# XinShuo-ph/gaussian_splatting_with_eye_tracking

Hardware: AMD Instinct MI355X
Metric: rendered views/sec (fwd+bwd) at 1080p, 1M Gaussians; achieved HBM GB/s % (higher is better)
Workload: dtype fp32; 1 GPU

## Files before the change

### gaussian_splatting_with_eye_tracking_amd/csrc/backward.hip

```cpp
#include <algorithm>

#include <hip/hip_ext.h>

#include "gs_blend.cuh"
#include "gs_blend_bwd.cuh"
#include "gs_bwd_math.cuh"
#include "gs_device.cuh"
#include "gs_kernels.h"

namespace gsamd {

constexpr int kDefaultBwdVariant = 2;
int g_bwd_variant = kDefaultBwdVariant;
void set_backward_variant(int v) { g_bwd_variant = v == 0 ? 0 : kDefaultBwdVariant; }

static BlendBwdParams blend_bwd_params(int W, int H, const ImageView& img, const BinningView& b, const GeomView& g,
                                       const float* colors, const float* bg, const float* dL_dpix) {
    return BlendBwdParams{W, H, img.ranges, img.max_contrib, b.point_list, reinterpret_cast<const float2*>(g.means2D),
                          reinterpret_cast<const float4*>(g.conic_opacity), colors, img.accum_alpha, img.n_contrib,
                          dL_dpix, bg, g.grad_accum, g_cull, (W + 15) / 16, img.bucket_count, img.bucket_list, g.hdr};
}

void launch_render_backward(int W, int H, const ImageView& img, const BinningView& b, const GeomView& g,
                            const float* colors, const float* bg, const float* dL_dpix, hipStream_t s) {
    const int gx = (W + 15) / 16, gy = (H + 15) / 16;
    if (gx == 0 || gy == 0) return;
    const BlendBwdParams p = blend_bwd_params(W, H, img, b, g, colors, bg, dL_dpix);
    const DispatchEvents ev = take_dispatch_events();
    if (g_bwd_variant == 0)
        hipExtLaunchKernelGGL(render_bwd_rows_kernel<BwdRows::kBase>, dim3(gx * gy), dim3(64), 0, s, ev.start, ev.stop,
                              0, p);
    else
        hipExtLaunchKernelGGL(render_bwd_kernel, dim3(gx * gy), dim3(64), 0, s, ev.start, ev.stop, 0, p);
}

constexpr uint32_t kDetNone = 0xffffffffu;
__global__ void __launch_bounds__(256) reduce_partials_kernel(
    int P, uint32_t R, uint32_t gx, uint32_t gy, const int* __restrict__ radii, const float2* __restrict__ means2D,
    const float* __restrict__ depths, const uint32_t* __restrict__ tiles_touched, const uint32_t* __restrict__ ranges,
    const uint32_t* __restrict__ max_contrib, const uint32_t* __restrict__ point_list,
    const float* __restrict__ partials, float* __restrict__ grad_accum, uint32_t* __restrict__ hdr,
    uint32_t err_token) {
    const int p = (int)((blockIdx.x * 256u + threadIdx.x) >> 4);
    const int sub = threadIdx.x & 15;
    if (p >= P) return;
    const int rad = radii[p];
    if (rad <= 0) return;
    const float2 xy = means2D[p];
    const Rect r = get_rect(xy.x, xy.y, rad, 16, 16, gx, gy);
    const uint32_t w = r.x1 - r.x0;
    const uint32_t area = w * (r.y1 - r.y0);
    const uint64_t key = ((uint64_t)float_bits(depths[p]) << 32) | (uint32_t)p;
    bool bad = area != tiles_touched[p];
    double acc = 0.0;
    if (!bad) {
        for (uint32_t i0 = 0; i0 < area; i0 += 16) {
            uint32_t pos = kDetNone;
            const uint32_t i = i0 + (uint32_t)sub;
            if (i < area) {
                const uint32_t tile = (r.y0 + i / w) * gx + r.x0 + i % w;
// ... 69 lines not shown
    const int idx = (int)(blockIdx.x * 256u + threadIdx.x);
    if (idx >= P || radii[idx] <= 0) return;
    float dz = grad_accum[(size_t)idx * kGradRow + kAuxDz];
    if (inv_depths) {
        const float f = inv_depth(inv_depths[idx]);
        dz = -(f * f) * dz;
    }
    dL_dmean3D[3 * idx + 0] += dz * viewmatrix[2];
    dL_dmean3D[3 * idx + 1] += dz * viewmatrix[6];
    dL_dmean3D[3 * idx + 2] += dz * viewmatrix[10];
}

void launch_aux_depth_to_means(int P, const GeomView& g, const int* radii, const float* viewmatrix,
                               float* dL_dmean3D, hipStream_t s, bool inverse) {
    if (P <= 0) return;
    hipLaunchKernelGGL(aux_depth_to_means_kernel, dim3(((unsigned)P + 255u) / 256u), dim3(256), 0, s, P, radii,
                       g.grad_accum, viewmatrix, dL_dmean3D, inverse ? g.depths : nullptr);
}

void launch_amr_render_backward(int W, int H, int mode, const ImageView& img, const BinningView& b,
                                const GeomView& g, const float* colors, const float* bg, const float* dL_dpix,
                                hipStream_t s) {
    const int tgx = (W + 31) / 32, tgy = (H + 31) / 32;
    if (tgx == 0 || tgy == 0 || mode == 0) return;
    BlendBwdParams p = blend_bwd_params(W, H, img, b, g, colors, bg, dL_dpix);
    p.amr_mode = mode;
    p.levels = img.levels;
    p.gx = tgx;
    hipLaunchKernelGGL(render_bwd_rows_kernel<BwdRows::kAmr>, dim3(4 * tgx * tgy), dim3(64), 0, s, p);
}


template <bool kHasSH, bool kHasScales, bool kSH16, bool kDrgb = false, bool kAA = false>
__device__ __forceinline__ void backward_gaussian_body(const BackwardGaussArgs& a,
                                                       const float* __restrict__ grad_accum,
                                                       const uint8_t* __restrict__ clamped_bits, int idx,
                                                       float* lrow, float (*small)[12] = nullptr,
                                                       float (*sh19)[19] = nullptr) {
    if (idx >= a.P) return;
    const bool vis = a.radii[idx] > 0;
    float acc[kNG];
    if (vis) {
        const float4* row = reinterpret_cast<const float4*>(grad_accum + (size_t)idx * kGradRow);
        const float4 r0 = row[0], r1 = row[1];
        const float r2 = grad_accum[(size_t)idx * kGradRow + 8];
        acc[0] = r0.x; acc[1] = r0.y; acc[2] = r0.z; acc[3] = r0.w;
        acc[4] = r1.x; acc[5] = r1.y; acc[6] = r1.z; acc[7] = r1.w; acc[8] = r2;
    } else {
#pragma unroll
        for (int q = 0; q < kNG; q++) acc[q] = 0.f;
    }
    if (a.err_word && (a.hdr[kHdrAntialias] != 0u) != kAA) {
        if (idx == 0) *a.err_word = a.err_token;
        if (vis) {
#pragma unroll
            for (int q = 0; q < kNG; q++) acc[q] = __uint_as_float(0x7fc00000u);
        }
    }
    if (small) {
        (*small)[9] = acc[0];
        (*small)[10] = acc[1];
        (*small)[11] = acc[2];
        (*small)[0] = acc[3];
        (*small)[1] = acc[4];
        (*small)[2] = 0.f;
    } else {
        if (a.dL_dcolor) {
            a.dL_dcolor[3 * idx + 0] = acc[0];
            a.dL_dcolor[3 * idx + 1] = acc[1];
            a.dL_dcolor[3 * idx + 2] = acc[2];
        }
        a.dL_dmean2D[3 * idx + 0] = acc[3];
        a.dL_dmean2D[3 * idx + 1] = acc[4];
        a.dL_dmean2D[3 * idx + 2] = 0.f;
    }
    if (a.dL_dconic) reinterpret_cast<float4*>(a.dL_dconic)[idx] = make_float4(acc[5], acc[6], 0.f, acc[7]);
    if constexpr (!kAA) store_out1(&a.dL_dopacity[idx], acc[8], a.nt_out != 0);

    const int ncoef_out = a.M;
    if (!vis) {
        if constexpr (kAA) store_out1(&a.dL_dopacity[idx], 0.f, a.nt_out != 0);
        if (small) {
#pragma unroll
            for (int i = 3; i < 9; i++) (*small)[i] = 0.f;
        } else {
#pragma unroll
            for (int i = 0; i < 3; i++) a.dL_dmean3D[3 * idx + i] = 0.f;
        }
        if (a.dL_dcov3D) {
#pragma unroll
            for (int i = 0; i < 6; i++) a.dL_dcov3D[6 * idx + i] = 0.f;
        }
        if (kDrgb) {
#pragma unroll
            for (int i = 0; i < 19; i++) (*sh19)[i] = 0.f;
        } else if (kHasSH && kSH16) {
#pragma unroll
            for (int i = 0; i < 48; i++) lrow[i] = 0.f;
        } else if (kHasSH) {
            for (int i = 0; i < ncoef_out * 3; i++) a.dL_dsh[(size_t)idx * ncoef_out * 3 + i] = 0.f;
        }
        if (!small)
            for (int i = 0; i < 3; i++) a.dL_dscale[3 * idx + i] = 0.f;
        for (int i = 0; i < 4; i++) a.dL_drot[4 * idx + i] = 0.f;
        return;
    }

    const float mx = a.means3D[3 * idx], my = a.means3D[3 * idx + 1], mz = a.means3D[3 * idx + 2];
    float cov3D[6];
    float4 qrot = make_float4(0.f, 0.f, 0.f, 0.f);
    float scl[3] = {0.f, 0.f, 0.f};
    if (kHasScales) {
        qrot = reinterpret_cast<const float4*>(a.rotations)[idx];
        scl[0] = a.scales[3 * idx + 0];
        scl[1] = a.scales[3 * idx + 1];
        scl[2] = a.scales[3 * idx + 2];
    }
    if (kHasScales && !a.has_cov_precomp) {
        compute_cov3d(scl, qrot, a.scale_modifier, cov3D);
    } else {
#pragma unroll
        for (int i = 0; i < 6; i++) cov3D[i] = a.cov3D[6 * idx + i];
    }
    float opac = 0.f;
    if constexpr (kAA) opac = a.opacities[idx];
    float s[16][3];
    uint8_t cb = 0;
    const bool use_drgb = kHasSH && a.drgb && a.hdr[kHdrDrgb] == 1u;
    float d9[9];
    if (kHasSH) {
        if (use_drgb) {
            const float4* row = reinterpret_cast<const float4*>(a.drgb) + 3 * (size_t)idx;
            const float4 r0 = row[0], r1 = row[1], r2 = row[2];
            d9[0] = r0.x; d9[1] = r0.y; d9[2] = r0.z; d9[3] = r0.w;
            d9[4] = r1.x; d9[5] = r1.y; d9[6] = r1.z; d9[7] = r1.w; d9[8] = r2.x;
        } else if constexpr (!kDrgb) {
            load_sh_rows<kSH16>(a, idx, s, lrow);
        } else {
// ... 42 lines not shown
        for (int c = 0; c < 3; c++) (*sh19)[16 + c] = dRGB[c];
    } else if (kHasSH) {
        if (use_drgb) sh_backward<kSH16>(a, idx, mx, my, mz, s, cb, acc, dmean, kSH16 ? lrow : nullptr, d9);
        else sh_backward<kSH16>(a, idx, mx, my, mz, s, cb, acc, dmean, kSH16 ? lrow : nullptr, nullptr);
    }
#pragma unroll
    for (int i = 0; i < 3; i++) {
        if (small) (*small)[3 + i] = dmean[i];
        else a.dL_dmean3D[3 * idx + i] = dmean[i];
    }

    if (kHasScales) {
        float dscale[3];
        float4 dq;
        cov3d_backward(qrot, scl, a.scale_modifier, dcov, dscale, dq);
        store_out4(reinterpret_cast<float4*>(a.dL_drot) + idx, dq, a.nt_out != 0);
        if (small) {
            (*small)[6] = dscale[0];
            (*small)[7] = dscale[1];
            (*small)[8] = dscale[2];
        } else {
            a.dL_dscale[3 * idx + 0] = dscale[0];
            a.dL_dscale[3 * idx + 1] = dscale[1];
            a.dL_dscale[3 * idx + 2] = dscale[2];
        }
    } else {
        if (small) {
            (*small)[6] = (*small)[7] = (*small)[8] = 0.f;
        } else {
            for (int i = 0; i < 3; i++) a.dL_dscale[3 * idx + i] = 0.f;
        }
        for (int i = 0; i < 4; i++) a.dL_drot[4 * idx + i] = 0.f;
    }
}

constexpr int kBgStageNt = 16;


template <bool kHasSH, bool kHasScales, bool kSH16, bool kSmall = false, bool kAA = false>
__global__ void __launch_bounds__(256) backward_gaussians_kernel(BackwardGaussArgs a, const float* __restrict__ grad_accum,
                                                                 const uint8_t* __restrict__ clamped_bits, int stage) {
    constexpr bool kStage = kHasSH && kSH16;
    static_assert(!kSmall || kStage, "the small outputs are staged in the SH rows' LDS");
    __shared__ float s_dsh[kStage ? 256 * kShRow : 1];
    const int idx = blockIdx.x * blockDim.x + threadIdx.x;
    if (kStage && !(a.drgb && a.hdr[kHdrDrgb] == 1u)) {
        const int g0 = blockIdx.x * blockDim.x;
        const int n = min(256, a.P - g0);
        const float4* in = reinterpret_cast<const float4*>(a.shs) + (size_t)g0 * 12;
        if (n == 256) {
            float4 v[12];
#pragma unroll
            for (int k = 0; k < 12; k++) v[k] = in[threadIdx.x + 256 * k];
#pragma unroll
            for (int k = 0; k < 12; k++) {
                const int f = threadIdx.x + 256 * k;
                float* r = s_dsh + (f / 12) * kShRow + 4 * (f % 12);
                r[0] = v[k].x; r[1] = v[k].y; r[2] = v[k].z; r[3] = v[k].w;
            }
        } else {
            for (int f = threadIdx.x; f < n * 12; f += 256) {
                const float4 v = in[f];
                float* r = s_dsh + (f / 12) * kShRow + 4 * (f % 12);
                r[0] = v.x; r[1] = v.y; r[2] = v.z; r[3] = v.w;
            }
        }
        __syncthreads();
    }
    float small[12];
    backward_gaussian_body<kHasSH, kHasScales, kSH16, false, kAA>(a, grad_accum, clamped_bits, idx,
                                                                  kStage ? s_dsh + threadIdx.x * kShRow : nullptr,
                                                                  kSmall ? &small : nullptr);
    if constexpr (kStage) {
        __syncthreads();
        const int g0 = blockIdx.x * blockDim.x;
        const int n = min(256, a.P - g0);
        float4* out = reinterpret_cast<float4*>(a.dL_dsh) + (size_t)g0 * 12;
        const bool nt = (stage & kBgStageNt) != 0;
        for (int f = threadIdx.x; f < n * 12; f += 256) {
            const float* r = s_dsh + (f / 12) * kShRow + 4 * (f % 12);
            store_out4(&out[f], make_float4(r[0], r[1], r[2], r[3]), nt);
        }
        if constexpr (kSmall) {
            __syncthreads();
            if (idx < a.P) {
#pragma unroll
                for (int i = 0; i < 12; i++) s_dsh[(i / 3) * 768 + 3 * threadIdx.x + i % 3] = small[i];
            }
            __syncthreads();
            const int nf = 3 * n;
            for (int f = threadIdx.x; f < 4 * 192; f += 256) {
                const int q = f / 192, i = f - 192 * q;
                float* d = q == 0 ? a.dL_dmean2D : q == 1 ? a.dL_dmean3D : q == 2 ? a.dL_dscale : a.dL_dcolor;
                if (!d || 4 * i >= nf) continue;
                const float* r = s_dsh + q * 768 + 4 * i;
                float* o = d + 3 * (size_t)g0 + 4 * i;
                if (4 * i + 4 <= nf) {
                    store_out4(reinterpret_cast<float4*>(o), make_float4(r[0], r[1], r[2], r[3]), a.nt_out != 0);
                } else {
                    for (int e = 0; e < 4 && 4 * i + e < nf; e++) o[e] = r[e];
                }
            }
        }
    }
}

template <bool kAA = false>
__global__ void __launch_bounds__(256) backward_gaussians_drgb_kernel(BackwardGaussArgs a,
                                                                      const float* __restrict__ grad_accum,
                                                                      const uint8_t* __restrict__ clamped_bits,
                                                                      int nt) {
    __shared__ float s_half[128 * kShRow];
    const int idx = blockIdx.x * blockDim.x + threadIdx.x;
    float small[12], sh19[19];
    backward_gaussian_body<true, true, true, true, kAA>(a, grad_accum, clamped_bits, idx, nullptr, &small, &sh19);
    const int g0 = blockIdx.x * blockDim.x;
    const int n = min(256, a.P - g0);
    const int ncoef = min((a.D + 1) * (a.D + 1), a.M);
#pragma unroll 1
    for (int h = 0; h < 2; h++) {
        const int gh = g0 + 128 * h, nh = min(128, n - 128 * h);
        if (nh <= 0) break;
        if (h) __syncthreads();
        if ((int)(threadIdx.x >> 7) == h && idx < a.P) {
            float* r = s_half + (threadIdx.x & 127) * kShRow;
#pragma unroll
            for (int k = 0; k < 16; k++)
#pragma unroll
                for (int c = 0; c < 3; c++) r[3 * k + c] = k < ncoef ? sh19[k] * sh19[16 + c] : 0.f;
        }
        __syncthreads();
        float4* out = reinterpret_cast<float4*>(a.dL_dsh) + (size_t)gh * 12;
        for (int f = threadIdx.x; f < nh * 12; f += 256) {
            const float* r = s_half + (f / 12) * kShRow + 4 * (f % 12);
            store_out4(&out[f], make_float4(r[0], r[1], r[2], r[3]), nt != 0);
        }
    }
    __syncthreads();
    if (idx < a.P) {
#pragma unroll
        for (int i = 0; i < 12; i++) s_half[(i / 3) * 768 + 3 * threadIdx.x + i % 3] = small[i];
    }
    __syncthreads();
    const int nf = 3 * n;
    for (int f = threadIdx.x; f < 4 * 192; f += 256) {
        const int q = f / 192, i = f - 192 * q;
        float* d = q == 0 ? a.dL_dmean2D : q == 1 ? a.dL_dmean3D : q == 2 ? a.dL_dscale : a.dL_dcolor;
        if (!d || 4 * i >= nf) continue;
        const float* r = s_half + q * 768 + 4 * i;
        float* o = d + 3 * (size_t)g0 + 4 * i;
        if (4 * i + 4 <= nf) {
            store_out4(reinterpret_cast<float4*>(o), make_float4(r[0], r[1], r[2], r[3]), a.nt_out != 0);
        } else {
            for (int e = 0; e < 4 && 4 * i + e < nf; e++) o[e] = r[e];
        }
    }
}

void launch_backward_gaussians(const BackwardGaussArgs& args, const GeomView& g, hipStream_t s) {
    if (args.P == 0) return;
    BackwardGaussArgs a = args;
    const dim3 grid((a.P + 255) / 256);
    const bool sh = a.shs != nullptr;
    const bool sh16 = sh && a.M == 16;
    const bool sc = a.scales != nullptr;
    a.nt_out = 0;
    const bool aa = a.antialiasing != 0;
#define GS_BG_LAUNCH(A, B, C)                                                                                      \
    do {                                                                                                           \
        if (aa)                                                                                                    \
            hipLaunchKernelGGL((backward_gaussians_kernel<A, B, C, false, true>), grid, dim3(256), 0, s, a,        \
                               g.grad_accum, g.clamped, 0);                                                        \
        else                                                                                                       \
            hipLaunchKernelGGL((backward_gaussians_kernel<A, B, C>), grid, dim3(256), 0, s, a, g.grad_accum,       \
                               g.clamped, 0);                                                                      \
    } while (0)
    if (sh16 && sc && a.drgb && a.drgb_known && a.P < 4000000) {
        if (aa)
            hipLaunchKernelGGL(backward_gaussians_drgb_kernel<true>, grid, dim3(256), 0, s, a, g.grad_accum,
                               g.clamped, 1);
        else
            hipLaunchKernelGGL(backward_gaussians_drgb_kernel<false>, grid, dim3(256), 0, s, a, g.grad_accum,
                               g.clamped, 1);
    } else if (sh16 && sc) {
        if (aa)
            hipLaunchKernelGGL((backward_gaussians_kernel<true, true, true, true, true>), grid, dim3(256), 0, s, a,
                               g.grad_accum, g.clamped, kBgStageNt);
        else
            hipLaunchKernelGGL((backward_gaussians_kernel<true, true, true, true>), grid, dim3(256), 0, s, a,
                               g.grad_accum, g.clamped, kBgStageNt);
    } else if (sh16) GS_BG_LAUNCH(true, false, true);
    else if (sh && sc) GS_BG_LAUNCH(true, true, false);
    else if (sh) GS_BG_LAUNCH(true, false, false);
    else if (sc) GS_BG_LAUNCH(false, true, false);
    else GS_BG_LAUNCH(false, false, false);
#undef GS_BG_LAUNCH
}

}
// ... 2 lines not shown
```

### gaussian_splatting_with_eye_tracking_amd/csrc/gs_api.cpp

```cpp
#include <hip/hip_runtime.h>

#include <atomic>
#include <cstdio>
#include <cstdlib>
#include <chrono>
#include <cstring>
#include <functional>
#include <algorithm>
#include <deque>
#include <mutex>
#include <stdexcept>
#include <string>
#include <unordered_set>
#include <utility>
#include <vector>

#include "../../include/gsplat_amd.h"
#include "gs_kernels.h"
#include "gs_layout.h"

using namespace gsamd;

namespace {

// ... 652 lines not shown

namespace {
size_t det_scratch_bytes(int R) { return R > 0 ? align_up(sizeof(float) * kDetRow * (size_t)R) : 0; }

struct DetScratch {
    bool on = false;
    char* base = nullptr;
    size_t bytes = 0;
};

void check_det_scratch(const DetScratch& d, int R, const char* who) {
    if (!d.on || R <= 0) return;
    if (!d.base) throw GsError(std::string(who) + ": scratch is NULL (gs_backward_deterministic_scratch_bytes)");
    if (d.bytes < det_scratch_bytes(R))
        throw GsError(std::string(who) + ": scratch of " + std::to_string(d.bytes) + " bytes, " +
                      std::to_string(det_scratch_bytes(R)) + " needed (gs_backward_deterministic_scratch_bytes)");
}

struct BackwardCall {
    BackwardGaussArgs a{};
    int R = 0, width = 0, height = 0;
    const float *background = nullptr, *colors_precomp = nullptr, *cov3D_precomp = nullptr, *dL_dpix = nullptr;
    char *geom_buffer = nullptr, *binning_buffer = nullptr, *img_buffer = nullptr;
    float* out_record = nullptr;
    DetScratch det;
    bool aux = false, inverse = false;
    const float *dL_ddepth = nullptr, *dL_dalpha = nullptr;
    int debug = 0;
    hipStream_t s = nullptr;
};

void blend_backward(const DetScratch& det, int width, int height, int P, int R, const ImageView& img,
                    const BinningView& b, const GeomView& g, const int* radii, const float* colors,
                    const float* background, const float* dL_dpix, int debug, hipStream_t s) {
    if (!det.on || R <= 0 || P <= 0) {
        zero_accum_unless_clean(g, P, s);
        if (R > 0 && P > 0) {
            StageTimer _t(kRenderBwd, s, true);
            launch_render_backward(width, height, img, b, g, colors, background, dL_dpix, s);
        }
        return;
    }
    take_accum_clean(g.grad_accum);
    const uint32_t token = next_error_token();
    {
        StageTimer _t(kRenderBwd, s);
        launch_render_backward_deterministic(width, height, P, R, img, b, g, radii, colors, background, dL_dpix,
                                             reinterpret_cast<float*>(det.base), token, s);
    }
    if (debug) {
        stage_check(true, s, "render_backward");
        uint32_t err = 0;
        GS_HIP(hipMemcpy(&err, g.hdr + kHdrError, sizeof(err), hipMemcpyDeviceToHost));
        if (err == token)
            throw GsError("deterministic backward: the geometry / binning / image buffers are not one forward's "
                          "(a Gaussian's tile rectangle and the sorted tile lists disagree)");
    }
}

int rasterizer_backward_impl(int amr_mode, const BackwardCall& c) {
    check_det_scratch(c.det, c.R, "gs_rasterizer_backward_deterministic");
    BackwardGaussArgs a = c.a;
    if (a.antialiasing && !a.opacities && a.P > 0)
        throw GsError("gs_rasterizer_backward_ex: the antialiased backward needs the forward's opacities");
    if (a.P <= 0) return 0;
    hipStream_t s = c.s;
    const Binned v = carve_buffers(c.geom_buffer, c.binning_buffer, c.img_buffer, a.P, c.R, c.width, c.height,
                                   amr_mode != 0 ? 32 : 16);
    const GeomView& g = v.g;
    if (!a.radii) a.radii = v.radii;
    const float* colors = c.colors_precomp ? c.colors_precomp : g.rgb;
    if (amr_mode != 0) {
        zero_accum_unless_clean(g, a.P, s);
        if (c.R > 0) {
            StageTimer _t(kRenderBwd, s);
            launch_amr_render_backward(c.width, c.height, amr_mode, v.img, v.b, g, colors, c.background, c.dL_dpix, s);
        }
    } else if (c.aux) {
        zero_accum_unless_clean(g, a.P, s);
        if (c.R > 0) {
            StageTimer _t(kRenderBwd, s, true);
            launch_render_backward_aux(c.width, c.height, v.img, v.b, g, colors, c.background, c.dL_dpix, c.dL_ddepth,
                                       c.dL_dalpha, s, c.inverse);
        }
    } else {
        blend_backward(c.det, c.width, c.height, a.P, c.R, v.img, v.b, g, a.radii, colors, c.background, c.dL_dpix,
                       c.debug, s);
    }
    stage_check(c.debug != 0, s, "render_backward");
    a.cov3D = c.cov3D_precomp ? c.cov3D_precomp : g.cov3D;
    a.has_cov_precomp = c.cov3D_precomp != nullptr;
    a.focal_y = (float)c.height / (2.0f * a.tan_fovy);
    a.focal_x = (float)c.width / (2.0f * a.tan_fovx);
    a.drgb = g.drgb;
    a.drgb_known = a.drgb != nullptr && drgb_written(g.drgb);
    a.hdr = g.hdr;
    a.err_word = g.hdr + kHdrError;
    a.err_token = next_error_token();
    { StageTimer _t(kBwdGauss, s); launch_backward_gaussians(a, g, s); }
    stage_check(c.debug != 0, s, "preprocess_backward");
    if (c.debug) {
        uint32_t err = 0;
        GS_HIP(hipMemcpy(&err, g.hdr + kHdrError, sizeof(err), hipMemcpyDeviceToHost));
        if (err == a.err_token)
            throw GsError(a.antialiasing
                              ? "backward: antialiasing is set but the forward that wrote these buffers was not "
                                "antialiased"
                              : "backward: the forward that wrote these buffers was antialiased; pass antialiasing "
                                "and its opacities (gs_rasterizer_backward_ex)");
    }
    if (c.aux && c.dL_ddepth && c.R > 0) {
        launch_aux_depth_to_means(a.P, g, a.radii, a.viewmatrix, a.dL_dmean3D, s, c.inverse);
        stage_check(c.debug != 0, s, "aux_depth_to_means");
    }
    return 0;
}

int backward_view_grads_impl(const BackwardCall& c, const char* who) {
    const BackwardGaussArgs& a = c.a;
    if (a.P < 0) throw GsError(std::string(who) + ": negative P");
    check_det_scratch(c.det, c.R, who);
// ... 748 lines not shown
}

int gs_activation_backward(int P, int M, int accumulate, const float* dL_dshs, const float* dL_dopacities,
                           const float* dL_dscales, const float* dL_drotations, const float* dL_dmeans3D,
                           const float* opacity_raw, const float* scaling_raw, const float* rotation_raw,
                           float* grad_xyz, float* grad_features_dc, float* grad_features_rest, float* grad_opacity,
                           float* grad_scaling, float* grad_rotation, void* stream) {
    return guarded([&]() -> int {
        if (P < 0 || M < 1 || M > 16) throw GsError("gs_activation_backward: bad sizes");
        hipStream_t s = static_cast<hipStream_t>(stream);
        launch_activation_backward(P, M, accumulate, dL_dshs, dL_dopacities, dL_dscales, dL_drotations, dL_dmeans3D,
                                   opacity_raw, scaling_raw, rotation_raw, grad_xyz, grad_features_dc,
                                   grad_features_rest, grad_opacity, grad_scaling, grad_rotation, s);
        stage_check(false, s, "activation_backward");
        return 0;
    });
}

namespace {
struct TuningKey {
    const char* key;
    const int* value;
    void (*set)(int);
};
const TuningKey kTuning[] = {
    {"fwd_variant", &g_fwd_variant, set_forward_variant},
    {"bwd_variant", &g_bwd_variant, set_backward_variant},
    {"amr_variant", &g_amr_variant, set_amr_variant},
    {"sort_algo", &g_sort_algo, set_sort_algo},
    {"cull", &g_cull, set_cull},
    {"hdr_mirror", &g_hdr_mirror, [](int v) { g_hdr_mirror = v == 0 ? 0 : 2; }},
    {"spec_dup", &g_spec_dup, [](int v) { g_spec_dup = v; }},
    {"fwd_fork", &g_fwd_fork, [](int v) { g_fwd_fork = v != 0; }},
    {"ritnet_mfma", &g_ritnet_mfma, set_ritnet_mfma},
};

const TuningKey* tuning_key(const char* key) {
    for (const TuningKey& e : kTuning)
        if (key && std::strcmp(key, e.key) == 0) return &e;
    if (key) g_err = std::string("unknown tuning key ") + key;
    return nullptr;
}
}

int gs_set_tuning(const char* key, int value) {
    const TuningKey* e = tuning_key(key);
    if (e) e->set(value);
    return e ? 0 : -1;
}

int gs_get_tuning(const char* key, int* value) {
    if (!key || !value) return -1;
    hdr_mirror_on();
    const TuningKey* e = tuning_key(key);
    if (!e) return -1;
    *value = *e->value;
    return 0;
}

int gs_set_thread_option(const char* key, int value) {
    if (!key) return -1;
    const struct { const char* key; int* value; } table[] = {{"fwd_no_grad", &t_fwd_no_grad},
                                                             {"sh_drgb", &t_sh_drgb},
                                                             {"store_cov3d", &t_store_cov3d},
                                                             {"fwd_zero", &t_fwd_zero},
                                                             {"amr_step0_unfilled", &t_amr_step0_unfilled}};
// ... 101 lines not shown
```

### gaussian_splatting_with_eye_tracking_amd/csrc/gs_blend_bwd.cuh

```cuda
#pragma once

#include <type_traits>

#include "gs_blend.cuh"
#include "gs_device.cuh"
#include "gs_kernels.h"

namespace gsamd {

constexpr int kNG = 9;
static_assert(kDetRow == kNG, "the deterministic backward's partial rows hold the nine terms");
constexpr int kAccRow = 9;
constexpr int kPPL = 4;
static_assert(kAuxDz == kAccRow && kAuxDz < kGradRow, "the aux backward's tenth sum takes a spare float of the row");
constexpr int kBwdBatch = 64;

struct BlendBwdParams {
    int W, H;
    const uint32_t *ranges, *max_contrib, *point_list;
    const float2* means2D;
    const float4* conic_opacity;
    const float *colors, *final_Ts;
    const uint32_t* n_contrib;
    const float *dL_dpixels, *bg;
    float* grad_accum;
    int cull, gx;
    const uint32_t *bucket_count, *bucket_list, *hdr;
    int amr_mode;
    const uint32_t* levels;
    const float *depths, *dL_ddepth, *dL_dalpha;
};

__device__ __forceinline__ float fma_dot3(float a0, float a1, float a2, float b0, float b1, float b2) {
    return __builtin_fmaf(a2, b2, __builtin_fmaf(a0, b0, a1 * b1));
}

__device__ __forceinline__ int bwd_block_tile(const uint32_t* __restrict__ bucket_count,
                                              const uint32_t* __restrict__ bucket_list, int lane) {
    int tile = (int)blockIdx.x;
    if (bucket_count) {
        const uint4 c4 = reinterpret_cast<const uint4*>(bucket_count)[lane];
        const uint32_t c = c4.x + c4.y + c4.z + c4.w;
        uint32_t incl = c;
#pragma unroll
        for (int d = 1; d < 64; d <<= 1) {
            const uint32_t y = (uint32_t)__shfl_up((int)incl, d, 64);
            if (lane >= d) incl += y;
        }
        const uint32_t rank = blockIdx.x;
        const uint64_t past = __ballot(incl > rank);
        const uint32_t total = (uint32_t)__builtin_amdgcn_readlane((int)incl, 63);
        if (total == gridDim.x && past != 0ull) {
            const int L = __builtin_ctzll(past);
            uint32_t r = rank - (uint32_t)__builtin_amdgcn_readlane((int)(incl - c), L);
            const uint32_t q0 = (uint32_t)__builtin_amdgcn_readlane((int)c4.x, L),
                           q1 = (uint32_t)__builtin_amdgcn_readlane((int)c4.y, L),
                           q2 = (uint32_t)__builtin_amdgcn_readlane((int)c4.z, L);
            int b = 4 * L;
            if (r >= q0) { r -= q0; b++;
                if (r >= q1) { r -= q1; b++;
                    if (r >= q2) { r -= q2; b++; } } }
            tile = (int)bucket_list[(size_t)b * gridDim.x + r];
        }
    }
// ... 47 lines not shown
                                                 uint32_t pstride) const {
        return use_codes ? code : cull ? splat_group_mask(xy, co, (float)ox, (float)oy, (float)pstride) : 0xfu;
    }
};

__device__ __forceinline__ uint64_t batch_masks(const uint64_t* s_bal, int top, uint32_t wave_last,
                                                const int (&group_last)[kPPL], uint64_t (&mk)[kPPL]) {
    const int j0 = __builtin_amdgcn_readfirstlane(max(0, top - (int)wave_last));
    uint64_t todo = 0;
    const uint64_t lo_cut = j0 >= 64 ? 0ull : j0 > 0 ? ~0ull << j0 : ~0ull;
#pragma unroll
    for (int k = 0; k < kPPL; k++) {
        const int jk = top - group_last[k];
        const uint64_t gcut = jk <= 0 ? ~0ull : (jk >= 64 ? 0ull : ~0ull << jk);
        mk[k] = uniform_u64(s_bal[k]) & lo_cut & gcut;
        todo |= mk[k];
    }
    return todo;
}

template <bool kOT>
__device__ __forceinline__ float flush_term(int fq, float qa, float sy, float4 pc, float ddelx_dx, float ddely_dy) {
#pragma clang fp contract(fast)
    const float o = kOT ? 1.0f : pc.w;
    const float cx = pc.x * (-1.0f / kHalfLog2e), cy = pc.y * (-1.0f / kLog2e), cz = pc.z * (-1.0f / kHalfLog2e);
    const float ka = fq == 3 ? -o * cx * ddelx_dx
                   : fq == 4 ? -o * cy * ddely_dy
                   : (fq >= 5 && fq <= 7) ? -0.5f * o
                   : (kOT && fq == 8) ? 1.0f / pc.w : 1.0f;
    const float kb = fq == 3 ? -o * cy * ddelx_dx : fq == 4 ? -o * cz * ddely_dy : 0.0f;
    return __builtin_fmaf(ka, qa, kb * sy);
}

__global__ void __launch_bounds__(64, 4) render_bwd_kernel(BlendBwdParams p) {
#pragma clang fp contract(fast)
    constexpr int kB = kBwdBatch;
    __shared__ uint32_t s_id[2][kB];
    __shared__ float4 s_a[kB];
    __shared__ float4 s_co[kB];
    __shared__ float4 s_b[kB];
    __shared__ uint64_t s_bal[4];
    constexpr int kStageSlots = 7;
    constexpr int kStagePitch = 272;
    __shared__ __attribute__((aligned(16))) float s_stage[3 * kStagePitch + 256];

    const int tid = threadIdx.x;
    const int lane = tid & 63;
    const int tile = bwd_block_tile(p.bucket_count, p.bucket_list, lane);
    const uint32_t ox = (uint32_t)(tile % p.gx) * 16, oy = (uint32_t)(tile / p.gx) * 16;
    const uint2 range = reinterpret_cast<const uint2*>(p.ranges)[tile];
    const int n = (int)(range.y - range.x);
    int m = min(n, (int)p.max_contrib[tile]);
    if (m == 0) return;

    const PixelSetT<kPPL> px = make_pixels_t<kPPL, 1>(p.W, p.H, ox, oy, 1);
    const float bg0 = p.bg[0], bg1 = p.bg[1], bg2 = p.bg[2];
    const float py0 = px.y[0];
    float T[kPPL], dpx[kPPL][3], acc_dot[kPPL];
    uint32_t last[kPPL];
    int group_last[kPPL];
    const uint32_t wave_last = load_pixel_state(p, px, true, T, last, dpx, group_last);
#pragma unroll
    for (int k = 0; k < kPPL; k++) acc_dot[k] = fma_dot3(bg0, bg1, bg2, dpx[k][0], dpx[k][1], dpx[k][2]);
    uint32_t min_last = 0xffffffffu;
#pragma unroll
    for (int k = 0; k < kPPL; k++) min_last = min(min_last, wave_min_u32(px.inside[k] ? last[k] : 0xffffffffu));
    min_last = (uint32_t)__builtin_amdgcn_readfirstlane((int)min_last);
// ... 123 lines not shown
                const float4 pc = s_co[j], cf = make_float4(a4.z, a4.w, s_b[j].x, 0.f);
                visit(j, xy, pc, cf, kFastT, kStartedT, kSlotT);
                nst = decltype(kSlotT)::value + 1;
            };
            while (todo) {
                one(std::integral_constant<int, 0>{});
                one(std::integral_constant<int, 1>{});
                one(std::integral_constant<int, 2>{});
                one(std::integral_constant<int, 3>{});
                one(std::integral_constant<int, 4>{});
                one(std::integral_constant<int, 5>{});
                one(std::integral_constant<int, 6>{});
                if (nst == kStageSlots) {
                    stage_reduce(kStageSlots, kFastT);
                    nst = 0;
                    js = 0ull;
                }
            }
            if (nst) stage_reduce(nst, kFastT);
            nst = 0;
        };
        const bool bsafe = (todo & ~fast_mask) == 0ull;
        if (bsafe && bstarted) run(T1{}, T1{});
        else if (bsafe) run(T1{}, T0{});
        else run(T0{}, T0{});
        __syncthreads();
        if (has_next) {
            s_id[par ^ 1][tid] = nr.id;
            nr.gather(p);
        }
    }
}

enum class BwdRows { kBase, kAmr, kDet, kAux, kAuxInv };

template <BwdRows kMode>
__global__ void __launch_bounds__(64, 4) render_bwd_rows_kernel(BlendBwdParams p) {
#pragma clang fp contract(fast)
    constexpr bool kAMR = kMode == BwdRows::kAmr, kDet = kMode == BwdRows::kDet;
    constexpr bool kInv = kMode == BwdRows::kAuxInv, kAux = kMode == BwdRows::kAux || kInv;
    constexpr int kRow = kAux ? kAccRow + 1 : kAccRow;
    constexpr int kB = kBwdBatch;
    __shared__ uint32_t s_id[2][kB];
    __shared__ float4 s_a[kB];
    __shared__ float4 s_co[kB];
    __shared__ float4 s_b[kB];
    __shared__ float s_acc[kB * kRow];
    __shared__ uint64_t s_bal[4];

    const int tid = threadIdx.x;
    const int lane = tid & 63;
    int tile;
    uint32_t ox, oy;
    constexpr uint32_t pstride = kAMR ? 2 : 1;
    if constexpr (kAMR) {
        tile = (int)(blockIdx.x >> 2);
        const uint32_t sx = blockIdx.x & 1u, sy = (blockIdx.x >> 1) & 1u;
        const uint32_t round = sx == 0 ? (sy == 0 ? 1u : 4u) : (sy == 0 ? 3u : 2u);
        const uint32_t L = min(p.levels[tile], 4u);
        if (p.amr_mode > 0 ? (round != (uint32_t)p.amr_mode || L < round) : round > L) return;
        ox = (uint32_t)(tile % p.gx) * 32 + sx;
        oy = (uint32_t)(tile / p.gx) * 32 + sy;
    } else {
        tile = bwd_block_tile(p.bucket_count, p.bucket_list, lane);
        ox = (uint32_t)(tile % p.gx) * 16;
        oy = (uint32_t)(tile / p.gx) * 16;
// ... 156 lines not shown
```

### gaussian_splatting_with_eye_tracking_amd/csrc/gs_kernels.h

```cpp
#pragma once

#include <hip/hip_runtime.h>
#include <stdint.h>

#include "gs_layout.h"

namespace gsamd {

struct DispatchEvents {
    hipEvent_t start = nullptr, stop = nullptr;
};
DispatchEvents take_dispatch_events();

struct PreprocessArgs {
    int P, D, M;
    const float* means3D;
    const float* scales;
    float scale_modifier;
    const float* rotations;
    const float* opacities;
    const float* shs;
    const float* cov3D_precomp;
    const float* colors_precomp;
    const float* viewmatrix;
// ... 27 lines not shown
constexpr int kLdsTiles = 16384;
void launch_count_tiles(int P, const GeomView& g, const int* radii, int W, int H, int block, const ImageView& img,
                        hipStream_t s);
void set_sort_algo(int v);
int bin_slots_for(int P, int gx, int gy, int block);
bool dup_banded(int gx, int gy, int block);
void launch_order_tiles(int T, const ImageView& img, bool use_max_contrib, hipStream_t s);
void launch_sort_tiles(int T, const ImageView& img, const BinningView& b, int max_count_host, int num_large_host,
                       hipStream_t s, int fused_max = 0);
constexpr int kAmrFusedSortMax = 2048;
constexpr int kAmrStepsAll = GSPLAT_AMD_AMR_STEPS_1_TO_4;
constexpr int kAmrStepsAllFill = GSPLAT_AMD_AMR_STEPS_1_TO_4_FILL;
constexpr int kAmrStepsAllSplit = GSPLAT_AMD_AMR_STEPS_1_TO_4_SPLIT;
constexpr int kAmrStateAfter = 100;
bool fused_sort_on();
void launch_reconstruct_keys(int T, const ImageView& img, const BinningView& b, const GeomView& g, uint64_t* keys,
                             hipStream_t s);

bool launch_render_forward(int W, int H, const ImageView& img, const BinningView& b, const GeomView& g,
                           const float* features, const float* bg, float* out_color, hipStream_t s,
                           float* zero_rows = nullptr, size_t zero_floats = 0, uint8_t* hit_codes = nullptr);
void launch_render_forward_aux(int W, int H, const ImageView& img, const BinningView& b, const GeomView& g,
                               float* out_depth, float* out_alpha, hipStream_t s, bool inverse = false);
void launch_render_backward_aux(int W, int H, const ImageView& img, const BinningView& b, const GeomView& g,
                                const float* colors, const float* bg, const float* dL_dpix, const float* dL_ddepth,
                                const float* dL_dalpha, hipStream_t s, bool inverse = false);
void launch_aux_depth_to_means(int P, const GeomView& g, const int* radii, const float* viewmatrix,
                               float* dL_dmean3D, hipStream_t s, bool inverse = false);
void set_forward_variant(int v);
void set_backward_variant(int v);
void set_amr_variant(int v);
void set_cull(int v);
void set_ritnet_mfma(int v);
void launch_render_backward(int W, int H, const ImageView& img, const BinningView& b, const GeomView& g,
                            const float* colors, const float* bg, const float* dL_dpix, hipStream_t s);
constexpr int kDetRow = 9;
void launch_render_backward_deterministic(int W, int H, int P, int R, const ImageView& img, const BinningView& b,
                                          const GeomView& g, const int* radii, const float* colors, const float* bg,
                                          const float* dL_dpix, float* partials, uint32_t err_token, hipStream_t s);

struct BackwardGaussArgs {
    int P, D, M;
    const float* means3D;
    const int* radii;
    const float* shs;
    const float* scales;
    const float* rotations;
    float scale_modifier;
    const float* cov3D;
    const float* viewmatrix;
    const float* projmatrix;
    const float* campos;
    float focal_x, focal_y, tan_fovx, tan_fovy;
    int has_cov_precomp;
    const float* drgb;
    const uint32_t* hdr;
    int drgb_known;
    int nt_out = 0;
    const float* opacities = nullptr;
    int antialiasing = 0;
    uint32_t* err_word = nullptr;
    uint32_t err_token = 0;
    float* dL_dmean2D;
    float* dL_dconic;
    float* dL_dopacity;
    float* dL_dcolor;
    float* dL_dmean3D;
    float* dL_dcov3D;
    float* dL_dsh;
    float* dL_dscale;
    float* dL_drot;
};
void launch_backward_gaussians(const BackwardGaussArgs& a, const GeomView& g, hipStream_t s);

constexpr int kViewRow = 10;
constexpr int kCamWords = 40;
constexpr int kMaxViews = 64;
struct MultiViewArgs {
    int P, D, M, V;
    int g0, count;
    const float* rows[kMaxViews];
    const float* cams[kMaxViews];
    const float* const* table;
    const float* means3D;
    const float* shs;
    const float* scales;
    const float* rotations;
    float scale_modifier;
    float* dL_dmean3D;
    float* dL_dsh;
    float* dL_dopacity;
    float* dL_dscale;
    float* dL_drot;
    float* grad_norm_accum;
    float* denom;
    float* max_radii;
    int nt = 0;
};
void launch_pack_view_grads(int P, const GeomView& g, const int* radii, bool has_sh, const float* viewmatrix,
                            const float* projmatrix, const float* campos, int width, int height, float tan_fovx,
                            float tan_fovy, float* out, hipStream_t s);
void launch_multiview_backward(const MultiViewArgs& a, hipStream_t s);

void launch_ritnet_conv(int k, const float* const* in_ptr, const int* in_c, const int* in_up, int nseg, int H, int W,
                        const float* w, const float* bias, int lrelu, const float* bn_scale, const float* bn_shift,
                        float* out, hipStream_t s);
// ... 58 lines not shown
```

Before: 1298 views/s.

## Zero gradient outputs inside blend backward tail and skip untouched Gaussians' stores

Adds a sparse-output path. The per-pixel blend backward kernel now zero-fills all per-Gaussian gradient output buffers in nontemporal slices after each tile's work. The per-Gaussian backward then treats Gaussians whose accumulated gradients are all zero as invisible, and skips writing their zeroed rows, tracking this with ballot-published live masks in LDS. The aim is to cut redundant HBM writes for Gaussians that touched no pixel, at the cost of extra zero-fill traffic inside the render backward kernel and more branching in the staged stores.

```diff
diff --git a/gaussian_splatting_with_eye_tracking_amd/csrc/backward.hip b/gaussian_splatting_with_eye_tracking_amd/csrc/backward.hip
--- a/gaussian_splatting_with_eye_tracking_amd/csrc/backward.hip
+++ b/gaussian_splatting_with_eye_tracking_amd/csrc/backward.hip
@@ -21,11 +21,30 @@
                           dL_dpix, bg, g.grad_accum, g_cull, (W + 15) / 16, img.bucket_count, img.bucket_list, g.hdr};
 }
 
+constexpr size_t kZeroWaveBudget = 64u << 10;
+bool plan_zero_segs(int W, int H, ZeroSegs& z) {
+    const size_t nb = (size_t)((W + 15) / 16) * (size_t)((H + 15) / 16);
+    size_t bytes = 0;
+    bool fits = nb > 0 && z.n > 0 && z.n <= kMaxZeroSegs;
+    for (int i = 0; fits && i < z.n; i++) {
+        bytes += sizeof(float) * (size_t)z.words[i];
+        fits = z.words[i] <= (1u << 31);
+        z.per[i] = (uint32_t)(((size_t)z.words[i] / 4 + nb - 1) / nb);
+    }
+    if (!fits || bytes > kZeroWaveBudget * nb) {
+        z.n = 0;
+        return false;
+    }
+    return true;
+}
+
 void launch_render_backward(int W, int H, const ImageView& img, const BinningView& b, const GeomView& g,
-                            const float* colors, const float* bg, const float* dL_dpix, hipStream_t s) {
+                            const float* colors, const float* bg, const float* dL_dpix, hipStream_t s,
+                            const ZeroSegs* zero) {
     const int gx = (W + 15) / 16, gy = (H + 15) / 16;
     if (gx == 0 || gy == 0) return;
-    const BlendBwdParams p = blend_bwd_params(W, H, img, b, g, colors, bg, dL_dpix);
+    BlendBwdParams p = blend_bwd_params(W, H, img, b, g, colors, bg, dL_dpix);
+    if (zero && g_bwd_variant != 0) p.zero = *zero;
     const DispatchEvents ev = take_dispatch_events();
     if (g_bwd_variant == 0)
         hipExtLaunchKernelGGL(render_bwd_rows_kernel<BwdRows::kBase>, dim3(gx * gy), dim3(64), 0, s, ev.start, ev.stop,
@@ -161,13 +180,13 @@
 
 
 template <bool kHasSH, bool kHasScales, bool kSH16, bool kDrgb = false, bool kAA = false>
-__device__ __forceinline__ void backward_gaussian_body(const BackwardGaussArgs& a,
+__device__ __forceinline__ bool backward_gaussian_body(const BackwardGaussArgs& a,
                                                        const float* __restrict__ grad_accum,
                                                        const uint8_t* __restrict__ clamped_bits, int idx,
                                                        float* lrow, float (*small)[12] = nullptr,
                                                        float (*sh19)[19] = nullptr) {
-    if (idx >= a.P) return;
-    const bool vis = a.radii[idx] > 0;
+    if (idx >= a.P) return false;
+    bool vis = a.radii[idx] > 0;
     float acc[kNG];
     if (vis) {
         const float4* row = reinterpret_cast<const float4*>(grad_accum + (size_t)idx * kGradRow);
@@ -186,6 +205,13 @@
             for (int q = 0; q < kNG; q++) acc[q] = __uint_as_float(0x7fc00000u);
         }
     }
+    if (a.skip_untouched && vis) {
+        uint32_t any = 0;
+#pragma unroll
+        for (int q = 0; q < kNG; q++) any |= float_bits(acc[q]);
+        vis = any != 0u;
+    }
+    const bool put = vis || !a.outputs_zeroed;
     if (small) {
         (*small)[9] = acc[0];
         (*small)[10] = acc[1];
@@ -203,12 +229,16 @@
         a.dL_dmean2D[3 * idx + 1] = acc[4];
         a.dL_dmean2D[3 * idx + 2] = 0.f;
     }
-    if (a.dL_dconic) reinterpret_cast<float4*>(a.dL_dconic)[idx] = make_float4(acc[5], acc[6], 0.f, acc[7]);
-    if constexpr (!kAA) store_out1(&a.dL_dopacity[idx], acc[8], a.nt_out != 0);
+    if (a.dL_dconic && put) reinterpret_cast<float4*>(a.dL_dconic)[idx] = make_float4(acc[5], acc[6], 0.f, acc[7]);
+    if constexpr (!kAA) {
+        if (put) store_out1(&a.dL_dopacity[idx], acc[8], a.nt_out != 0);
+    }
 
     const int ncoef_out = a.M;
     if (!vis) {
-        if constexpr (kAA) store_out1(&a.dL_dopacity[idx], 0.f, a.nt_out != 0);
+        if constexpr (kAA) {
+            if (put) store_out1(&a.dL_dopacity[idx], 0.f, a.nt_out != 0);
+        }
         if (small) {
 #pragma unroll
             for (int i = 3; i < 9; i++) (*small)[i] = 0.f;
@@ -216,7 +246,7 @@
 #pragma unroll
             for (int i = 0; i < 3; i++) a.dL_dmean3D[3 * idx + i] = 0.f;
         }
-        if (a.dL_dcov3D) {
+        if (a.dL_dcov3D && put) {
 #pragma unroll
             for (int i = 0; i < 6; i++) a.dL_dcov3D[6 * idx + i] = 0.f;
         }
@@ -231,8 +261,9 @@
         }
         if (!small)
             for (int i = 0; i < 3; i++) a.dL_dscale[3 * idx + i] = 0.f;
-        for (int i = 0; i < 4; i++) a.dL_drot[4 * idx + i] = 0.f;
-        return;
+        if (put)
+            for (int i = 0; i < 4; i++) a.dL_drot[4 * idx + i] = 0.f;
+        return false;
     }
 
     const float mx = a.means3D[3 * idx], my = a.means3D[3 * idx + 1], mz = a.means3D[3 * idx + 2];
@@ -341,9 +372,36 @@
         }
         for (int i = 0; i < 4; i++) a.dL_drot[4 * idx + i] = 0.f;
     }
+    return true;
 }
 
 constexpr int kBgStageNt = 16;
+
+__device__ __forceinline__ void publish_live(uint64_t* s_live, bool live) {
+    const uint64_t m = __ballot(live);
+    if ((threadIdx.x & 63u) == 0u) s_live[threadIdx.x >> 6] = m;
+}
+__device__ __forceinline__ bool row_live(const uint64_t* s_live, int r) { return (s_live[r >> 6] >> (r & 63)) & 1ull; }
+
+__device__ __forceinline__ void store_small_staged(const BackwardGaussArgs& a, const float* s, int g0, int n,
+                                                   const uint64_t* s_live) {
+    const bool sparse = a.outputs_zeroed != 0;
+    const int nf = 3 * n;
+    for (int f = threadIdx.x; f < 4 * 192; f += 256) {
+        const int q = f / 192, i = f - 192 * q;
+        float* d = q == 0 ? a.dL_dmean2D : q == 1 ? a.dL_dmean3D : q == 2 ? a.dL_dscale : a.dL_dcolor;
+        if (!d || 4 * i >= nf) continue;
+        const float* r = s + q * 768 + 4 * i;
+        float* o = d + 3 * (size_t)g0 + 4 * i;
+        if (4 * i + 4 <= nf) {
+            if (sparse && !row_live(s_live, (4 * i) / 3) && !row_live(s_live, (4 * i + 3) / 3)) continue;
+            store_out4(reinterpret_cast<float4*>(o), make_float4(r[0], r[1], r[2], r[3]), a.nt_out != 0);
+        } else {
+            for (int e = 0; e < 4 && 4 * i + e < nf; e++)
+                if (!sparse || row_live(s_live, (4 * i + e) / 3)) o[e] = r[e];
+        }
+    }
+}
 
 
 template <bool kHasSH, bool kHasScales, bool kSH16, bool kSmall = false, bool kAA = false>
@@ -352,6 +410,7 @@
     constexpr bool kStage = kHasSH && kSH16;
     static_assert(!kSmall || kStage, "the small outputs are staged in the SH rows' LDS");
     __shared__ float s_dsh[kStage ? 256 * kShRow : 1];
+    __shared__ uint64_t s_live[4];
     const int idx = blockIdx.x * blockDim.x + threadIdx.x;
     if (kStage && !(a.drgb && a.hdr[kHdrDrgb] == 1u)) {
         const int g0 = blockIdx.x * blockDim.x;
@@ -377,16 +436,18 @@
         __syncthreads();
     }
     float small[12];
-    backward_gaussian_body<kHasSH, kHasScales, kSH16, false, kAA>(a, grad_accum, clamped_bits, idx,
-                                                                  kStage ? s_dsh + threadIdx.x * kShRow : nullptr,
-                                                                  kSmall ? &small : nullptr);
+    const bool live = backward_gaussian_body<kHasSH, kHasScales, kSH16, false, kAA>(
+        a, grad_accum, clamped_bits, idx, kStage ? s_dsh + threadIdx.x * kShRow : nullptr, kSmall ? &small : nullptr);
     if constexpr (kStage) {
+        const bool sparse = kSmall && a.outputs_zeroed != 0;
+        publish_live(s_live, live);
         __syncthreads();
         const int g0 = blockIdx.x * blockDim.x;
         const int n = min(256, a.P - g0);
         float4* out = reinterpret_cast<float4*>(a.dL_dsh) + (size_t)g0 * 12;
         const bool nt = (stage & kBgStageNt) != 0;
         for (int f = threadIdx.x; f < n * 12; f += 256) {
+            if (sparse && !row_live(s_live, f / 12)) continue;
             const float* r = s_dsh + (f / 12) * kShRow + 4 * (f % 12);
             store_out4(&out[f], make_float4(r[0], r[1], r[2], r[3]), nt);
         }
@@ -397,19 +458,7 @@
                 for (int i = 0; i < 12; i++) s_dsh[(i / 3) * 768 + 3 * threadIdx.x + i % 3] = small[i];
             }
             __syncthreads();
-            const int nf = 3 * n;
-            for (int f = threadIdx.x; f < 4 * 192; f += 256) {
-                const int q = f / 192, i = f - 192 * q;
-                float* d = q == 0 ? a.dL_dmean2D : q == 1 ? a.dL_dmean3D : q == 2 ? a.dL_dscale : a.dL_dcolor;
-                if (!d || 4 * i >= nf) continue;
-                const float* r = s_dsh + q * 768 + 4 * i;
-                float* o = d + 3 * (size_t)g0 + 4 * i;
-                if (4 * i + 4 <= nf) {
-                    store_out4(reinterpret_cast<float4*>(o), make_float4(r[0], r[1], r[2], r[3]), a.nt_out != 0);
-                } else {
-                    for (int e = 0; e < 4 && 4 * i + e < nf; e++) o[e] = r[e];
-                }
-            }
+            store_small_staged(a, s_dsh, g0, n, s_live);
         }
     }
 }
@@ -420,9 +469,13 @@
                                                                       const uint8_t* __restrict__ clamped_bits,
                                                                       int nt) {
     __shared__ float s_half[128 * kShRow];
+    __shared__ uint64_t s_live[4];
     const int idx = blockIdx.x * blockDim.x + threadIdx.x;
     float small[12], sh19[19];
-    backward_gaussian_body<true, true, true, true, kAA>(a, grad_accum, clamped_bits, idx, nullptr, &small, &sh19);
+    const bool live =
+        backward_gaussian_body<true, true, true, true, kAA>(a, grad_accum, clamped_bits, idx, nullptr, &small, &sh19);
+    const bool sparse = a.outputs_zeroed != 0;
+    publish_live(s_live, live);
     const int g0 = blockIdx.x * blockDim.x;
     const int n = min(256, a.P - g0);
     const int ncoef = min((a.D + 1) * (a.D + 1), a.M);
@@ -441,6 +494,7 @@
         __syncthreads();
         float4* out = reinterpret_cast<float4*>(a.dL_dsh) + (size_t)gh * 12;
         for (int f = threadIdx.x; f < nh * 12; f += 256) {
+            if (sparse && !row_live(s_live, 128 * h + f / 12)) continue;
             const float* r = s_half + (f / 12) * kShRow + 4 * (f % 12);
             store_out4(&out[f], make_float4(r[0], r[1], r[2], r[3]), nt != 0);
         }
@@ -451,19 +505,11 @@
         for (int i = 0; i < 12; i++) s_half[(i / 3) * 768 + 3 * threadIdx.x + i % 3] = small[i];
     }
     __syncthreads();
-    const int nf = 3 * n;
-    for (int f = threadIdx.x; f < 4 * 192; f += 256) {
-        const int q = f / 192, i = f - 192 * q;
-        float* d = q == 0 ? a.dL_dmean2D : q == 1 ? a.dL_dmean3D : q == 2 ? a.dL_dscale : a.dL_dcolor;
-        if (!d || 4 * i >= nf) continue;
-        const float* r = s_half + q * 768 + 4 * i;
-        float* o = d + 3 * (size_t)g0 + 4 * i;
-        if (4 * i + 4 <= nf) {
-            store_out4(reinterpret_cast<float4*>(o), make_float4(r[0], r[1], r[2], r[3]), a.nt_out != 0);
-        } else {
-            for (int e = 0; e < 4 && 4 * i + e < nf; e++) o[e] = r[e];
-        }
-    }
+    store_small_staged(a, s_half, g0, n, s_live);
+}
+
+bool backward_gaussians_sparse_form(const BackwardGaussArgs& a) {
+    return a.shs != nullptr && a.M == 16 && a.scales != nullptr;
 }
 
 void launch_backward_gaussians(const BackwardGaussArgs& args, const GeomView& g, hipStream_t s) {
@@ -474,6 +520,7 @@
     const bool sh16 = sh && a.M == 16;
     const bool sc = a.scales != nullptr;
     a.nt_out = 0;
+    if (!backward_gaussians_sparse_form(a)) a.outputs_zeroed = 0;
     const bool aa = a.antialiasing != 0;
 #define GS_BG_LAUNCH(A, B, C)                                                                                      \
     do {                                                                                                           \
diff --git a/gaussian_splatting_with_eye_tracking_amd/csrc/gs_api.cpp b/gaussian_splatting_with_eye_tracking_amd/csrc/gs_api.cpp
--- a/gaussian_splatting_with_eye_tracking_amd/csrc/gs_api.cpp
+++ b/gaussian_splatting_with_eye_tracking_amd/csrc/gs_api.cpp
@@ -708,12 +708,13 @@
 
 void blend_backward(const DetScratch& det, int width, int height, int P, int R, const ImageView& img,
                     const BinningView& b, const GeomView& g, const int* radii, const float* colors,
-                    const float* background, const float* dL_dpix, int debug, hipStream_t s) {
+                    const float* background, const float* dL_dpix, int debug, hipStream_t s,
+                    const ZeroSegs* zero = nullptr) {
     if (!det.on || R <= 0 || P <= 0) {
         zero_accum_unless_clean(g, P, s);
         if (R > 0 && P > 0) {
             StageTimer _t(kRenderBwd, s, true);
-            launch_render_backward(width, height, img, b, g, colors, background, dL_dpix, s);
+            launch_render_backward(width, height, img, b, g, colors, background, dL_dpix, s, zero);
         }
         return;
     }
@@ -732,6 +733,32 @@
             throw GsError("deterministic backward: the geometry / binning / image buffers are not one forward's "
                           "(a Gaussian's tile rectangle and the sorted tile lists disagree)");
     }
+}
+
+int g_bwd_sparse = 1;
+
+bool sparse_outputs(const BackwardCall& c, const BackwardGaussArgs& a, int amr_mode, ZeroSegs& z) {
+    z = ZeroSegs{};
+    if (!g_bwd_sparse || amr_mode != 0 || c.aux || c.det.on || g_bwd_variant == 0 || c.R <= 0 || c.width <= 0 ||
+        c.height <= 0 || !backward_gaussians_sparse_form(a))
+        return false;
+    const struct { float* p; size_t per_gaussian; } outs[kMaxZeroSegs] = {
+        {a.dL_dmean2D, 3}, {a.dL_dconic, 4}, {a.dL_dopacity, 1},           {a.dL_dcolor, 3}, {a.dL_dmean3D, 3},
+        {a.dL_dcov3D, 6},  {a.dL_dsh, 3 * (size_t)a.M}, {a.dL_dscale, 3}, {a.dL_drot, 4}};
+    for (const auto& o : outs) {
+        const size_t words = o.per_gaussian * (size_t)a.P;
+        if (!o.p) continue;
+        if (words > (1u << 31)) return false;
+        z.ptr[z.n] = o.p;
+        z.words[z.n] = (uint32_t)words;
+        z.n++;
+    }
+    if (z.n == 0) return false;
+    if (!plan_zero_segs(c.width, c.height, z)) {
+        for (const auto& o : outs)
+            if (o.p) GS_HIP(hipMemsetAsync(o.p, 0, sizeof(float) * o.per_gaussian * (size_t)a.P, c.s));
+    }
+    return true;
 }
 
 int rasterizer_backward_impl(int amr_mode, const BackwardCall& c) {
@@ -760,9 +787,12 @@
                                        c.dL_dalpha, s, c.inverse);
         }
     } else {
+        ZeroSegs zero;
+        a.outputs_zeroed = sparse_outputs(c, a, amr_mode, zero);
         blend_backward(c.det, c.width, c.height, a.P, c.R, v.img, v.b, g, a.radii, colors, c.background, c.dL_dpix,
-                       c.debug, s);
-    }
+                       c.debug, s, zero.n ? &zero : nullptr);
+    }
+    a.skip_untouched = g_bwd_sparse != 0;
     stage_check(c.debug != 0, s, "render_backward");
     a.cov3D = c.cov3D_precomp ? c.cov3D_precomp : g.cov3D;
     a.has_cov_precomp = c.cov3D_precomp != nullptr;
@@ -1577,6 +1607,7 @@
     {"hdr_mirror", &g_hdr_mirror, [](int v) { g_hdr_mirror = v == 0 ? 0 : 2; }},
     {"spec_dup", &g_spec_dup, [](int v) { g_spec_dup = v; }},
     {"fwd_fork", &g_fwd_fork, [](int v) { g_fwd_fork = v != 0; }},
+    {"bwd_sparse", &g_bwd_sparse, [](int v) { g_bwd_sparse = v != 0; }},
     {"ritnet_mfma", &g_ritnet_mfma, set_ritnet_mfma},
 };
 
diff --git a/gaussian_splatting_with_eye_tracking_amd/csrc/gs_blend_bwd.cuh b/gaussian_splatting_with_eye_tracking_amd/csrc/gs_blend_bwd.cuh
--- a/gaussian_splatting_with_eye_tracking_amd/csrc/gs_blend_bwd.cuh
+++ b/gaussian_splatting_with_eye_tracking_amd/csrc/gs_blend_bwd.cuh
@@ -29,7 +29,31 @@
     int amr_mode;
     const uint32_t* levels;
     const float *depths, *dL_ddepth, *dL_dalpha;
+    ZeroSegs zero;
 };
+
+__device__ __forceinline__ void zero_fill_slices(const ZeroSegs& z, uint32_t lane) {
+    typedef float f4v __attribute__((ext_vector_type(4)));
+    const uint32_t r = blockIdx.x;
+#pragma unroll
+    for (int i = 0; i < kMaxZeroSegs; i++) {
+        if (i < z.n) {
+            float* const d = z.ptr[i];
+            const uint32_t w = z.words[i];
+            const uint32_t head = min(w, (uint32_t)((16u - ((uintptr_t)d & 15u)) & 15u) >> 2);
+            const uint32_t nv = (w - head) >> 2;
+            const uint64_t lo64 = (uint64_t)r * z.per[i];
+            const uint32_t lo = (uint32_t)min((uint64_t)nv, lo64), hi = (uint32_t)min((uint64_t)nv, lo64 + z.per[i]);
+            f4v* const v = reinterpret_cast<f4v*>(d + head);
+            for (uint32_t k = lo + lane; k < hi; k += 64) __builtin_nontemporal_store(f4v{0.f, 0.f, 0.f, 0.f}, v + k);
+            if (r == 0) {
+                const uint32_t t0 = head + 4u * nv;
+                if (lane < head) d[lane] = 0.f;
+                if (lane >= 4u && lane - 4u < w - t0) d[t0 + lane - 4u] = 0.f;
+            }
+        }
+    }
+}
 
 __device__ __forceinline__ float fma_dot3(float a0, float a1, float a2, float b0, float b1, float b2) {
     return __builtin_fmaf(a2, b2, __builtin_fmaf(a0, b0, a1 * b1));
@@ -143,7 +167,7 @@
     return __builtin_fmaf(ka, qa, kb * sy);
 }
 
-__global__ void __launch_bounds__(64, 4) render_bwd_kernel(BlendBwdParams p) {
+__device__ __forceinline__ void render_bwd_tile(const BlendBwdParams& p) {
 #pragma clang fp contract(fast)
     constexpr int kB = kBwdBatch;
     __shared__ uint32_t s_id[2][kB];
@@ -333,6 +357,11 @@
     }
 }
 
+__global__ void __launch_bounds__(64, 4) render_bwd_kernel(BlendBwdParams p) {
+    render_bwd_tile(p);
+    if (p.zero.n != 0) zero_fill_slices(p.zero, threadIdx.x);
+}
+
 enum class BwdRows { kBase, kAmr, kDet, kAux, kAuxInv };
 
 template <BwdRows kMode>
diff --git a/gaussian_splatting_with_eye_tracking_amd/csrc/gs_kernels.h b/gaussian_splatting_with_eye_tracking_amd/csrc/gs_kernels.h
--- a/gaussian_splatting_with_eye_tracking_amd/csrc/gs_kernels.h
+++ b/gaussian_splatting_with_eye_tracking_amd/csrc/gs_kernels.h
@@ -83,8 +83,17 @@
 void set_amr_variant(int v);
 void set_cull(int v);
 void set_ritnet_mfma(int v);
+constexpr int kMaxZeroSegs = 9;
+struct ZeroSegs {
+    float* ptr[kMaxZeroSegs];
+    uint32_t words[kMaxZeroSegs];
+    uint32_t per[kMaxZeroSegs];
+    int n;
+};
 void launch_render_backward(int W, int H, const ImageView& img, const BinningView& b, const GeomView& g,
-                            const float* colors, const float* bg, const float* dL_dpix, hipStream_t s);
+                            const float* colors, const float* bg, const float* dL_dpix, hipStream_t s,
+                            const ZeroSegs* zero = nullptr);
+bool plan_zero_segs(int W, int H, ZeroSegs& z);
 constexpr int kDetRow = 9;
 void launch_render_backward_deterministic(int W, int H, int P, int R, const ImageView& img, const BinningView& b,
                                           const GeomView& g, const int* radii, const float* colors, const float* bg,
@@ -112,6 +121,8 @@
     int antialiasing = 0;
     uint32_t* err_word = nullptr;
     uint32_t err_token = 0;
+    int skip_untouched = 0;
+    int outputs_zeroed = 0;
     float* dL_dmean2D;
     float* dL_dconic;
     float* dL_dopacity;
@@ -123,6 +134,7 @@
     float* dL_drot;
 };
 void launch_backward_gaussians(const BackwardGaussArgs& a, const GeomView& g, hipStream_t s);
+bool backward_gaussians_sparse_form(const BackwardGaussArgs& a);
 
 constexpr int kViewRow = 10;
 constexpr int kCamWords = 40;
```

Result: no change. 1303 views/s (median of 6 runs) (+0.4%).
